# samuelskirvin/EIGENSOLVER

Hardware: AMD Instinct MI355X
Metric: det(M) evals/sec + roots/sec, 4096x4096 (k,omega) grid (higher is better)
Workload: dtype f64

## Files before the change

eigensolver_amd/build.py:

```python
import os
import shutil
import subprocess
import sys

HERE = os.path.dirname(os.path.abspath(__file__))
CSRC = os.path.join(HERE, "csrc")
LIBDIR = os.path.join(HERE, "lib")
LIB = os.path.join(LIBDIR, "libeigensolver_amd.so")
LIB_IEEE = os.path.join(LIBDIR, "libeigensolver_amd_ieee.so")
PROBE_SRC = os.path.join(os.path.dirname(HERE), "tests", "devmath", "devmath_probe.hip")
LIB_PROBE = os.path.join(LIBDIR, "libes_devmath_probe.so")
ARCH = "gfx950"
FLAGS = ["-O3", "-fPIC", "-std=c++17", f"--offload-arch={ARCH}", "-ffp-contract=off", "-fno-fast-math",
         "-Wall", "-Wno-unused-function", "-Wno-unused-result"]


def _hipcc():
    for c in (os.environ.get("HIPCC"), shutil.which("hipcc"), "/opt/rocm/bin/hipcc"):
        if c and os.path.exists(c):
            return c
    raise RuntimeError("hipcc not found (ROCm toolchain required)")


def sources():
    return sorted(os.path.join(CSRC, f) for f in os.listdir(CSRC) if f.endswith(".hip"))


def _deps():
    out = sources() + [os.path.join(CSRC, f) for f in os.listdir(CSRC) if f.endswith((".hpp", ".h"))]
    out.append(os.path.join(os.path.dirname(HERE), "include", "eigensolver_amd.h"))
    return out


def needs_build(lib=LIB):
    if not os.path.exists(lib):
        return True
    t = os.path.getmtime(lib)
    return any(os.path.getmtime(s) > t for s in _deps())


def _compile_and_link(lib, extra_flags, tag, verbose):
    hipcc = _hipcc()
    objs = []
    procs = []
    for src in sources():
        obj = os.path.join(LIBDIR, os.path.basename(src)[:-4] + tag + ".o")
        cmd = [hipcc] + FLAGS + extra_flags + ["-c", src, "-o", obj]
        if verbose:
            print(" ".join(cmd))
        procs.append((src, subprocess.Popen(cmd, stdout=subprocess.PIPE, stderr=subprocess.STDOUT, text=True)))
        objs.append(obj)
    for src, p in procs:
        out, _ = p.communicate()
        if p.returncode != 0:
            raise RuntimeError(f"hipcc failed for {src}:\n{out}")
        if verbose and out.strip():
            print(out)
    cmd = [hipcc, "-shared", "-fPIC", f"--offload-arch={ARCH}", "-o", lib] + objs
    r = subprocess.run(cmd, stdout=subprocess.PIPE, stderr=subprocess.STDOUT, text=True)
    if r.returncode != 0:
        raise RuntimeError(f"link failed:\n{r.stdout}")
    return lib


def _probe_needs_build():
    if not os.path.exists(LIB_PROBE):
        return True
    t = os.path.getmtime(LIB_PROBE)
    return any(os.path.getmtime(s) > t for s in (PROBE_SRC, os.path.join(CSRC, "es_bessel.hpp")))


def _build_probe(verbose):
    cmd = [_hipcc()] + FLAGS + ["-shared", PROBE_SRC, "-o", LIB_PROBE]
    if verbose:
        print(" ".join(cmd))
    r = subprocess.run(cmd, stdout=subprocess.PIPE, stderr=subprocess.STDOUT, text=True)
    if r.returncode != 0:
        raise RuntimeError(f"hipcc failed for {PROBE_SRC}:\n{r.stdout}")
    if verbose and r.stdout.strip():
        print(r.stdout)


def build(force=False, verbose=False):
    os.makedirs(LIBDIR, exist_ok=True)
    extra = ["-DES_ALL_GRID_SHAPES"] if os.environ.get("ES_BUILD_ALL_SHAPES") == "1" else []
    extra += os.environ.get("ES_BUILD_EXTRA_FLAGS", "").split()
    if force or needs_build(LIB):
        _compile_and_link(LIB, extra, "", verbose)
    if force or needs_build(LIB_IEEE):
        _compile_and_link(LIB_IEEE, ["-DES_IEEE_DIVISION"], ".ieee", verbose)
    if os.path.exists(PROBE_SRC) and (force or _probe_needs_build()):
        _build_probe(verbose)
    return LIB


if __name__ == "__main__":
    print(build(force="--force" in sys.argv, verbose=True))
```

eigensolver_amd/csrc/es_bessel.hpp:

```cpp
#pragma once
#include <math.h>

#ifndef ES_HD
#if defined(__HIPCC__)
#define ES_HD __host__ __device__ __forceinline__
#else
#define ES_HD static inline
#endif
#endif

namespace esb {

ES_HD double qdiv(double a, double b) {
#if defined(__HIP_DEVICE_COMPILE__) && !defined(ES_IEEE_DIVISION)
  const double r0 = __builtin_amdgcn_rcp(b);
  const double e = __builtin_fma(-b, r0, 1.0);
  const double t = __builtin_fma(e, e, e);
  return a * __builtin_fma(r0, t, r0);
#else
  return a / b;
#endif
}

#if defined(__HIP_DEVICE_COMPILE__) && !defined(ES_IEEE_DIVISION)
#define ES_BESSEL_TABLES 1
#define ES_R(k) (1.0 / (double)(k))
#define ES_R8(k) ES_R(k), ES_R((k) + 1), ES_R((k) + 2), ES_R((k) + 3), ES_R((k) + 4), ES_R((k) + 5), ES_R((k) + 6), ES_R((k) + 7)
#define ES_A(i) (1.0 / (-(((double)(i)) - 0.5) * (((double)(i)) - 0.5)))
#define ES_A8(i) ES_A(i), ES_A((i) + 1), ES_A((i) + 2), ES_A((i) + 3), ES_A((i) + 4), ES_A((i) + 5), ES_A((i) + 6), ES_A((i) + 7)
constexpr int kRcpTable = 64;
static __constant__ double kRcpInt[kRcpTable] = {0.0, ES_R(1), ES_R(2), ES_R(3), ES_R(4), ES_R(5), ES_R(6), ES_R(7), ES_R8(8), ES_R8(16),
                                                 ES_R8(24), ES_R8(32), ES_R8(40), ES_R8(48), ES_R8(56)};
static __constant__ double kRcpCF2a[kRcpTable] = {0.0, ES_A(1), ES_A(2), ES_A(3), ES_A(4), ES_A(5), ES_A(6), ES_A(7), ES_A8(8), ES_A8(16),
                                                  ES_A8(24), ES_A8(32), ES_A8(40), ES_A8(48), ES_A8(56)};
#undef ES_R
#undef ES_R8
#undef ES_A
#undef ES_A8
#endif

ES_HD double qdiv_int(double a, int k) {
#if defined(ES_BESSEL_TABLES)
  if (k < kRcpTable) return a * kRcpInt[k];
#endif
  return qdiv(a, (double)k);
}
ES_HD double qdiv_cf2a(double a, int i, double ai) {
#if defined(ES_BESSEL_TABLES)
  if (i < kRcpTable) return a * kRcpCF2a[i];
#endif
  return qdiv(a, ai);
}

constexpr double kEulerGamma = 0.57721566490153286060651209008240243;
constexpr double kPi = 3.14159265358979323846264338327950288;

#define ES_CHEB_K0 { \
    1.2201515410329777, -0.0314481013119645, 0.0015698838857300533, -0.00012849549581627802, \
    1.39498137188765e-05, -1.8317555227191195e-06, 2.766813639445015e-07, -4.660489897687948e-08, \
    8.574034017414225e-09, -1.6975345093890614e-09, 3.5773972814003283e-10, -7.957489244477396e-11, \
    1.8559491149549264e-11, -4.514597883374519e-12, 1.1403405882073441e-12, -2.9800969231481784e-13, \
    8.032890775068375e-14, -2.2275133267462965e-14, 6.340076476276646e-15, -1.848593377920907e-15, \
    5.5120559994043335e-16, -1.6782311257549006e-16, 5.2103917776435543e-17, -1.6475805939842632e-17, \
    5.3004337711773354e-18 }
#define ES_CHEB_K1 { \
    1.3603130952422213, 0.10392373657681724, -0.002857816859622779, 0.00019521551847135162, \
    -1.936197974166083e-05, 2.406484947837217e-06, -3.5019606030878126e-07, 5.7410841254500495e-08, \
    -1.0345762465678097e-08, 2.0150497551970347e-09, -4.1903547593419254e-10, 9.218315187605315e-11, \
    -2.129967838427791e-11, 5.139639673482343e-12, -1.2891739609498229e-12, 3.348419666052243e-13, \
    -8.976705182010146e-14, 2.4771544242195988e-14, -7.0198370892147685e-15, 2.038703166239861e-15, \
    -6.057047270643018e-16, 1.8380935752430455e-16, -5.689462849193648e-17, 1.7940510478863572e-17, \
    -5.7567444820733025e-18 }
constexpr int kChebN = 25;
#if defined(__HIP_DEVICE_COMPILE__)
static __constant__ double kChebK0[kChebN] = ES_CHEB_K0;
static __constant__ double kChebK1[kChebN] = ES_CHEB_K1;
#else
static const double kChebK0[kChebN] = ES_CHEB_K0;
static const double kChebK1[kChebN] = ES_CHEB_K1;
#endif

ES_HD void ke01(double x, double& k0, double& k1) {
  if (x <= 2.0) {
    const double t = 0.25 * x * x;
    const double lg = log(0.5 * x) + kEulerGamma;
    double term0 = 1.0, i0 = 1.0, s0 = 0.0, hk = 0.0;
    double term1 = 1.0, i1 = 1.0, s1 = 1.0;
    for (int k = 1; k < 40; ++k) {
      const double rk = qdiv_int(1.0, k), rk1 = qdiv_int(1.0, k + 1);
      term0 = term0 * t * (rk * rk);
      hk += rk;
      i0 += term0;
      s0 += hk * term0;
      term1 = term1 * t * (rk * rk1);
      i1 += term1;
      s1 += (hk + hk + rk1) * term1;
      if (term0 < 1e-18 * i0) break;
    }
    const double ex = exp(x);
    k0 = ex * (-lg * i0 + s0);
    k1 = ex * (qdiv(1.0, x) + lg * (0.5 * x) * i1 - 0.25 * x * s1);
  } else {
    const double y = qdiv(4.0, x) - 1.0, y2 = y + y;
    double p1 = 0.0, p2 = 0.0, q1 = 0.0, q2 = 0.0;
#pragma unroll
    for (int j = kChebN - 1; j >= 1; --j) {
      const double pn = fma(y2, p1, kChebK0[j] - p2);
      const double qn = fma(y2, q1, kChebK1[j] - q2);
      p2 = p1; p1 = pn;
      q2 = q1; q1 = qn;
    }
    const double rs = qdiv(1.0, sqrt(x));
    k0 = fma(y, p1, kChebK0[0] - p2) * rs;
    k1 = fma(y, q1, kChebK1[0] - q2) * rs;
  }
}

ES_HD void ke_pair(int n, double x, double& kn, double& knp1) {
  double a, b;
  ke01(x, a, b);
  const double tox = qdiv(2.0, x);
  for (int j = 1; j <= n; ++j) {
    const double c = a + (double)j * tox * b;
    a = b;
    b = c;
  }
  kn = a;
  knp1 = b;
}

ES_HD void ie_pair(int n, double x, double& in_, double& inp1) {
  const double t = 0.25 * x * x;
  const double hx = 0.5 * x;
  double pre = 1.0;
  for (int j = 1; j <= n; ++j) pre *= hx / (double)j;
  double term_a = 1.0, sum_a = 1.0;
  double term_b = 1.0, sum_b = 1.0;
  for (int k = 1; k < 400; ++k) {
    const double kk = (double)k;
    term_a = term_a * t / (kk * (kk + (double)n));
    term_b = term_b * t / (kk * (kk + (double)n + 1.0));
    sum_a += term_a;
    sum_b += term_b;
    if (term_a < 1e-18 * sum_a) break;
  }
  const double ex = exp(-x);
  in_ = ex * pre * sum_a;
  inp1 = ex * pre * (hx / ((double)n + 1.0)) * sum_b;
}

ES_HD void ie_pair_from_k(int n, double x, double kn, double knp1, double& in_, double& inp1) {
  if (x < 0.5) { ie_pair(n, x, in_, inp1); return; }
  const int M = n + 10 + (int)sqrt(40.0 * x);
  const double tox = 2.0 / x;
  double ip = 0.0, ic = 1e-200;
  double ktox = (double)M * tox;
  for (int k = M; k > n; --k) {
    const double im = fma(ktox, ic, ip);
    ip = ic;
    ic = im;
    ktox -= tox;
  }
  const double f = ip / ic;
  in_ = 1.0 / (x * fma(f, kn, knp1));
  inp1 = f * in_;
}

ES_HD void jy_pair(int n, double x, double& jn, double& jn1, double& yn, double& yn1) {
  int M = (int)(1.15 * x) + 36 + n;
  M += (M & 1);
  const double tox = 2.0 / x;
  double jp = 0.0, jc = 1e-280;
  double norm = 0.0, sy0 = 0.0, sy1 = 0.0;
  double rn = 0.0, rn1 = 0.0;
  for (int k = M; k >= 1; --k) {
    if (k == n) rn = jc;
    if (k == n + 1) rn1 = jc;
    const int h = k >> 1;
    const double sgn = (h & 1) ? -1.0 : 1.0;
    if ((k & 1) == 0) {
      norm += jc;
      sy0 -= sgn * jc / (double)h;
    } else if (k >= 3) {
      sy1 += sgn * (double)k * jc / ((double)h * (double)(h + 1));
    }
    const double jm = (double)k * tox * jc - jp;
    jp = jc;
    jc = jm;
    if (fabs(jc) > 1e250) {
      const double sc = 1e-250;
      jc *= sc; jp *= sc; norm *= sc; sy0 *= sc; sy1 *= sc; rn *= sc; rn1 *= sc;
    }
  }
  if (n == 0) rn = jc;
  if (n + 1 == 1) rn1 = jp;
  const double inv = 1.0 / (jc + 2.0 * norm);
  const double j0 = jc * inv, j1 = jp * inv;
  const double lg = log(0.5 * x) + kEulerGamma;
  const double y0 = (2.0 / kPi) * (lg * j0 + 2.0 * sy0 * inv);
// ... 15 lines not shown
```

eigensolver_amd/csrc/es_shoot.hip:

```cpp
#include <vector>
#include <cstdio>
#include <cstdlib>
#include <cmath>
#include <type_traits>

#include "es_shoot_shared.hpp"

namespace {
using namespace es_shoot_shared;

struct GridOpts {
  int skip;
  const int* cols;
  int part;
  int main_span;
};

constexpr long ES_TILE_GRID_X = 1L << 22;
__device__ __forceinline__ long es_tile_index() { return (long)blockIdx.y * ES_TILE_GRID_X + blockIdx.x; }
inline dim3 es_tile_grid(long tiles) {
  return tiles <= ES_TILE_GRID_X ? dim3((unsigned)tiles) : dim3((unsigned)ES_TILE_GRID_X, (unsigned)((tiles + ES_TILE_GRID_X - 1) / ES_TILE_GRID_X));
}

template <int FAM, int PTS, int MAXT, bool TRACK, int WPE = 0>
// ... 66 lines not shown
    const int j = (int)(c - row * nw);
    if (!dead[j]) continue;
    const double k = kv[row];
    const double w = k * wv[j];
    const double k2 = k * k;
    const double Oe = (P.family == FAM_CYL0 || P.family == FAM_CYLT) ? w : (w - k * P.U_e);
    const double Oe2 = Oe * Oe;
    const double m_e = ((k2 * P.vAe2 - Oe2) * (k2 * P.ce2 - Oe2)) / (P.Se * (k2 * P.cTe2 - Oe2));
    const double cst = (P.family == FAM_CYL0 || P.family == FAM_CYLT)
                           ? -1.0 / (P.rho_e * (k2 * P.vAe2 - w * w))
                           : P.rho_e * P.Se * (k2 * P.cTe2 - Oe2) / (Oe * (k2 * P.ce2 - Oe2));
    uint8_t st = ES_PT_CONTINUUM;
    if (m_e < 0.0) st = ES_PT_LEAKY;
    else if (!(m_e > 0.0) || !isfinite(m_e) || !isfinite(cst)) st = ES_PT_NONFINITE;
    Dout[c] = NAN;
    if (relout) relout[c] = NAN;
    stout[c] = st;
  }
}

template <int FAM>
__global__ __launch_bounds__(256) void shoot_points_kernel(ShootDev P, const double* __restrict__ kv,
                                                           const double* __restrict__ wv, const int* __restrict__ d_n,
                                                           int n_max, double* __restrict__ Dout,
                                                           double* __restrict__ relout, uint8_t* __restrict__ stout) {
  ES_POINT_LDS(FAM);
  const int n = es_count(d_n, n_max);
  if ((long)blockIdx.x * 256 >= (long)n) return;
  const int i = blockIdx.x * blockDim.x + threadIdx.x;
  const bool in = i < n;
  const double k = in ? kv[i] : 1.0;
  const double w = in ? wv[i] : 1.0;
  double D, rel; uint8_t st;
  shoot_point<FAM>(P, k, w, w, D, rel, st, es_point_lds);
  if (in) {
    Dout[i] = D;
    stout[i] = st;
    if (relout) relout[i] = rel;
  }
}

__global__ __launch_bounds__(256) void bracket_flag_kernel(const double* __restrict__ D,
                                                           const uint8_t* __restrict__ st, int nw, long cells,
                                                           uint64_t* __restrict__ masks,
                                                           int* __restrict__ block_counts) {
  __shared__ int wave_cnt[4];
  const long c = (long)blockIdx.x * 256 + threadIdx.x;
  const int lane = threadIdx.x & 63;
  double d0 = 0.0; int ok0 = 0;
  if (c < cells) { d0 = D[c]; ok0 = (st[c] == ES_PT_OK); }
  double d1 = __shfl_down(d0, 1);
  int ok1 = __shfl_down(ok0, 1);
  if (lane == 63) {
    if (c + 1 < cells) { d1 = D[c + 1]; ok1 = (st[c + 1] == ES_PT_OK); } else { d1 = 0.0; ok1 = 0; }
  }
  bool flag = false;
  if (c < cells) {
    const long row = c / nw;
    const int j = (int)(c - row * nw);
    flag = (j < nw - 1) && ok0 && ok1 && (d0 * d1 < 0.0);
  }
  const uint64_t m = __ballot(flag);
  if (lane == 0) {
    masks[c >> 6] = m;
    wave_cnt[threadIdx.x >> 6] = __popcll(m);
  }
  __syncthreads();
// ... 1690 lines not shown
```

eigensolver_amd/csrc/es_shoot_device.hpp:

```cpp
#pragma once
#include <hip/hip_runtime.h>
#include <math.h>
#include "es_bessel.hpp"
#include "../../include/eigensolver_amd.h"

enum { FAM_CYL0 = 0, FAM_CYLT = 1, FAM_SLABD = 2, FAM_SLABF = 3 };

struct ShootDev {
  int family;
  int n_nodes;
  int npts;
  double xb;
  double h;
  const double* base;
  double rho_e, vAe2, ce2, cTe2, Se, U_e;
  double R_factor;
  double ic0, ic1;
  int m, m_ext, axis_bc, c1_power;
  double bc_const;
  double bc_const_raw;
  double slab_sign;
  double c2_i, vA2_i, S_i, cT2_i, rho_i;
  int accept_norm;
  int use_bands, n_bands;
// ... 302 lines not shown
}

template <int FAM>
__device__ __forceinline__ void adjoint_step(double& p, double& q, const Coef& B0, const Coef& Bm, const Coef& B1,
                                             double h, double h2, double h6, double h3) {
  if (fam_unnormalised<FAM>()) rk4_step_adjoint_scaled0_x3(p, q, B0, Bm, B1);
  else if (fam_scaled<FAM>()) rk4_step_adjoint_scaled0(p, q, B0, Bm, B1);
  else rk4_step_adjoint<FamTraits<FAM>::SHAPE>(p, q, B0, Bm, B1, h, h2, h6, h3);
}

template <int FAM>
__device__ __forceinline__ void adjoint_step_normalised(double& p, double& q, const Coef& B0, const Coef& Bm, const Coef& B1,
                                                        double h, double h2, double h6, double h3) {
  if (fam_scaled<FAM>()) rk4_step_adjoint_scaled0(p, q, B0, Bm, B1);
  else rk4_step_adjoint<FamTraits<FAM>::SHAPE>(p, q, B0, Bm, B1, h, h2, h6, h3);
}

__device__ __forceinline__ void adjoint_start(const ShootDev& P, const Coef& A_last, double& p, double& q) {
  if ((P.family == FAM_CYL0 || P.family == FAM_CYLT) && P.axis_bc == ES_AXIS_SAUSAGE) {
    p = A_last.a11; q = A_last.a12;
  } else {
    p = 1.0; q = 0.0;
  }
}

struct Exterior {
  double m_e;
  double cst;
  double yb, dyb;
  double Oe;
  int status;
};

__device__ __forceinline__ Exterior exterior_cylinder(const ShootDev& P, double k, double w, double w_cst) {
  Exterior X;
  const double k2 = k * k, w2 = w * w;
  X.Oe = w;
  X.m_e = ((k2 * P.vAe2 - w2) * (k2 * P.ce2 - w2)) / (P.Se * (k2 * P.cTe2 - w2));
  X.cst = -1.0 / (P.rho_e * (k2 * P.vAe2 - w_cst * w_cst));
  X.yb = X.dyb = NAN;
  if (X.m_e < 0.0) { X.status = ES_PT_LEAKY; return X; }
  if (!(X.m_e > 0.0) || !isfinite(X.m_e) || !isfinite(X.cst)) { X.status = ES_PT_NONFINITE; return X; }
  X.status = ES_PT_OK;
  const double mu = sqrt(X.m_e);
  const double sgn = (P.xb < 0.0) ? -1.0 : 1.0;
  const double xR = mu * (P.R_factor / k), xb = mu;
  const int n = P.m_ext;
  double Kb, Kb1, KR, KR1;
  esb::ke_pair(n, xb, Kb, Kb1);
  esb::ke_pair(n, xR, KR, KR1);
  const double dn = (double)n;
  const double dKb = -Kb1 + (dn / xb) * Kb;
  const double dKR = -KR1 + (dn / xR) * KR;
  const double g = P.ic1 / (sgn * mu);
  double Pv, dPv;
  const double gap = xR - xb;
  if (gap < 40.0) {
    double Ib, Ib1, IR, IR1;
    esb::ie_pair_from_k(n, xb, Kb, Kb1, Ib, Ib1);
    esb::ie_pair_from_k(n, xR, KR, KR1, IR, IR1);
    const double dIb = Ib1 + (dn / xb) * Ib;
    const double dIR = IR1 + (dn / xR) * IR;
    const double a_s = -(P.ic0 * dKR - g * KR);
    const double b_s = -(g * IR - P.ic0 * dIR);
    const double E2 = exp(-2.0 * gap);
    Pv = b_s * Kb + E2 * a_s * Ib;
    dPv = sgn * mu * (b_s * dKb + E2 * a_s * dIb);
  } else {
    double IR, IR1;
    const double rI = 1.0 - 0.5 / xR - (4.0 * dn * dn - 1.0) / (8.0 * xR * xR);
    (void)IR; (void)IR1;
    const double b_s = -(g - P.ic0 * rI);
    Pv = b_s * Kb;
    dPv = sgn * mu * (b_s * dKb);
  }
  const double nrm = fabs(Pv);
  X.yb = Pv / nrm;
  X.dyb = dPv / nrm;
  if (!isfinite(X.yb) || !isfinite(X.dyb)) X.status = ES_PT_NONFINITE;
  return X;
}

__device__ __forceinline__ Exterior exterior_slab(const ShootDev& P, double k, double w) {
  Exterior X;
  const double k2 = k * k;
  const double Oe = w - k * P.U_e;
  const double Oe2 = Oe * Oe;
  X.Oe = Oe;
  X.m_e = ((k2 * P.vAe2 - Oe2) * (k2 * P.ce2 - Oe2)) / (P.Se * (k2 * P.cTe2 - Oe2));
  X.cst = P.rho_e * P.Se * (k2 * P.cTe2 - Oe2) / (Oe * (k2 * P.ce2 - Oe2));
  X.yb = X.dyb = NAN;
  if (X.m_e < 0.0) { X.status = ES_PT_LEAKY; return X; }
  if (!(X.m_e > 0.0) || !isfinite(X.m_e) || !isfinite(X.cst)) { X.status = ES_PT_NONFINITE; return X; }
  X.status = ES_PT_OK;
  const double mu = sqrt(X.m_e);
  const double R = P.R_factor / k;
  const double E2 = exp(-2.0 * mu * (R - 1.0));
  const double gp = P.ic0 + P.ic1 / mu, gm = P.ic0 - P.ic1 / mu;
  const double V = gp + E2 * gm;
  const double dV = mu * (gp - E2 * gm);
  const double nrm = fabs(V);
  X.yb = V / nrm;
  X.dyb = dV / nrm;
  if (!isfinite(X.yb) || !isfinite(X.dyb)) X.status = ES_PT_NONFINITE;
  return X;
}

struct Mismatch { double d, outer, inner; };

template <int FAM, class Ext>
__device__ __forceinline__ Mismatch boundary_algebra(const ShootDev& P, const KScal& s, double w, const Ext& X,
                                                     double r1, double r2, const double* e_first) {
  Mismatch M;
  if (FAM == FAM_CYL0 || FAM == FAM_CYLT) {
    const double Pb = X.yb;
    const double xi_e = X.outer;
    double Xb;
    if (P.axis_bc == ES_AXIS_KINK) {
      Xb = (P.bc_const * xi_e - r1 * Pb) / r2;
    } else if (P.axis_bc == ES_AXIS_ROTATION_KINK) {
      Xb = (-(P.bc_const * xi_e) - r1 * Pb) / r2;
    } else {
      Xb = -(r1 * Pb) / r2;
    }
    const double xi_i = Xb / P.xb;
    M.outer = xi_e; M.inner = xi_i; M.d = xi_e - xi_i;
  } else {
    const double P_left = X.outer;
    if (FAM == FAM_SLABD) {
      const double Vb = X.yb;
      const double sv = (P.slab_sign - r1) * Vb / r2;
      M.inner = sv / w;
    } else {
      const double Omb = w - e_first[0];
      const double Vb = X.yb * Omb / X.Oe;
      const double sv = (P.slab_sign - r1) * Vb / r2;
      const double Omb2 = Omb * Omb;
      const double PTi = P.rho_i * P.S_i * (s.kcT2 - Omb2) / (Omb * (s.kc2 - Omb2));
      M.inner = PTi * sv;
    }
    M.outer = P_left;
    M.d = P_left - M.inner;
  }
  return M;
}
```

eigensolver_amd/csrc/es_shoot_grid_body.hpp:

```cpp
  constexpr int NE = FamTraits<FAM>::NE;
  constexpr int LSTRIDE = 2 * CH + 2;
  constexpr bool PAIR = (FAM == FAM_CYL0) && !TRACK;
  constexpr bool STASH = (WPE != 0);
  __shared__ double xstash[STASH ? 4 * PTS * MAXT : 1];
  __shared__ __attribute__((aligned(16))) double lds_all[ROWS * NE * LSTRIDE];
  const int TW = blockDim.x;
  const int T = TW / ROWS;
  const int sub = (ROWS == 2 && (int)threadIdx.x >= T) ? 1 : 0;
  const int tl = (int)threadIdx.x - sub * T;
  const int tb = (ROWS == 2) ? sub * (NE * LSTRIDE) : 0;
  const int nsteps = P.n_nodes - 1;
  const double h = P.h, h2 = 0.5 * P.h, h6 = P.h / 6.0, h3 = P.h / 3.0;

  const int span = T * PTS;
  const int ncols = opts.cols ? opts.cols[0] : nw;
  const int col_base = (opts.part == 2) ? (ncols / opts.main_span) * opts.main_span : 0;
  const int nseg = (opts.part == 2) ? opts.main_span / span : (nw + span - 1) / span;
  const int ngroups = (nk + ROWS - 1) / ROWS;
  const long ntiles = (long)ngroups * nseg;
  for (long tile = es_tile_index(), once = 1; once && tile < ntiles; once = 0) {
    const int seg = (int)(tile / ngroups);
    const int grp = (int)(tile - (long)seg * ngroups);
    const bool row_ok = (ROWS == 1) || grp * ROWS + sub < nk;
    const int row = (ROWS == 1) ? grp : (row_ok ? grp * ROWS + sub : nk - 1);
    const int w0 = col_base + seg * span;
    if (w0 >= ncols) continue;
    if (opts.part == 1 && w0 + span > ncols) continue;
    const double k = kv[row];
    const KScal s = make_kscal(P, k);
    {
      double w[PTS], zp[PTS], zq[PTS];
      Coef B0[PTS], B1[PTS];
      SignTrack trk[PTS];
      bool inr[PTS];
      int iwp[PTS];
      ExteriorLite X[PTS];
      bool lane_live = false;
      if (STASH) {
#pragma unroll 1
        for (int p = 0; p < PTS; ++p) {
          const int ic = w0 + p * T + tl;
          const bool in = row_ok && ic < ncols;
          const int iw = in ? (opts.cols ? opts.cols[1 + ic] : ic) : 0;
          const double wp = in ? pick_w(wv, w_mode, k, row, nw, iw) : 1.0;
          const ExteriorLite Xp = exterior_lite(P, k, wp, wp);
          const bool dead = opts.skip && !TRACK && band_crossed(P, k, wp);
          lane_live = lane_live || (in && Xp.status == ES_PT_OK && !dead);
          double* xs = xstash + (size_t)(4 * p) * MAXT + threadIdx.x;
          xs[0] = Xp.outer; xs[MAXT] = Xp.yb; xs[2 * MAXT] = Xp.Oe; xs[3 * MAXT] = (double)Xp.status;
        }
      }
#pragma unroll
      for (int p = 0; p < PTS; ++p) {
        const int ic = w0 + p * T + tl;
        inr[p] = row_ok && ic < ncols;
        iwp[p] = inr[p] ? (opts.cols ? opts.cols[1 + ic] : ic) : 0;
        w[p] = inr[p] ? pick_w(wv, w_mode, k, row, nw, iwp[p]) : 1.0;
      }
      if (!STASH) {
#pragma unroll
        for (int p = 0; p < PTS; ++p) {
          X[p] = exterior_lite(P, k, w[p], w[p]);
          const bool dead = opts.skip && !TRACK && band_crossed(P, k, w[p]);
          lane_live = lane_live || (inr[p] && X[p].status == ES_PT_OK && !dead);
        }
      }
      const bool wave_live = __any(lane_live);
      const bool wg_live = __syncthreads_or(wave_live ? 1 : 0) != 0;
#pragma unroll
      for (int p = 0; p < PTS; ++p) { zp[p] = 0.0; zq[p] = 0.0; }
      const int nchunks = wg_live ? (nsteps + CH - 1) / CH : 0;
      for (int c = nchunks - 1; c >= 0; --c) {
        const int c0 = c * CH;
        const int nst = (nsteps - c0 < CH) ? (nsteps - c0) : CH;
        __syncthreads();
        const int nstage = 2 * nst + ES_FAR_NODE(c, nchunks);
        for (int i = threadIdx.x; i < ROWS * nstage; i += TW) {
          double b[FamTraits<FAM>::NB], e[NE];
          const int r = (ROWS == 2 && i >= nstage) ? 1 : 0;
          const int node = i - r * nstage;
          load_base<FAM>(P, 2 * c0 + node, b);
          if (ROWS == 1) {
            make_entry<FAM, fam_scaled<FAM>()>(b, s, e);
          } else {
            const int rr = grp * ROWS + r;
            const KScal sr = make_kscal(P, kv[rr < nk ? rr : nk - 1]);
            make_entry<FAM, fam_scaled<FAM>()>(b, sr, e);
          }
#pragma unroll
          for (int f = 0; f < NE; ++f) lds_all[r * (NE * LSTRIDE) + f * LSTRIDE + node] = e[f];
        }
        __syncthreads();
        if (!wave_live) continue;
        if (c == nchunks - 1) {
          double eL[NE];
// ... 67 lines not shown
            for (int p = 0; p < PTS; ++p) B0[p] = B1[p];
            --j;
          }
          for (; j >= 1; j -= 2) {
            ES_MARCH_STEP(j, B0, B1)
            ES_MARCH_STEP(j - 1, B1, B0)
          }
        } else {
          for (; j >= 0; --j) {
            ES_MARCH_STEP(j, B0, B1)
#pragma unroll
            for (int p = 0; p < PTS; ++p) B0[p] = B1[p];
          }
        }
#undef ES_MARCH_PAIR
#undef ES_MARCH_STEP
#pragma unroll
        for (int p = 0; p < PTS; ++p) adjoint_rescale<FAM>(zp[p], zq[p], nsteps - c0 - nst, nsteps - c0);
      }
      if (STASH) {
#pragma unroll
        for (int p = 0; p < PTS; ++p) {
          const double* xs = xstash + (size_t)(4 * p) * MAXT + threadIdx.x;
          X[p].outer = xs[0]; X[p].yb = xs[MAXT]; X[p].Oe = xs[2 * MAXT]; X[p].status = (int)xs[3 * MAXT];
        }
      }
      double bf[FamTraits<FAM>::NB], ef[NE];
      load_base<FAM>(P, 0, bf);
      make_entry<FAM>(bf, s, ef);
#pragma unroll
      for (int p = 0; p < PTS; ++p) {
        if (!inr[p]) continue;
        const int iw = iwp[p];
        const Mismatch M = boundary_algebra<FAM>(P, s, w[p], X[p], zp[p], zq[p], ef);
        double D, rel; uint8_t st;
        const bool crossed = TRACK ? trk[p].crossed() : band_crossed(P, k, w[p]);
        finish_point(P, M, X[p], crossed, D, rel, st);
        if (opts.skip && !TRACK && crossed && X[p].status == ES_PT_OK) st = ES_PT_CONTINUUM;
        if (opts.skip && st == ES_PT_CONTINUUM) { D = NAN; rel = NAN; }
        const size_t o = (size_t)row * nw + iw;
        Dout[o] = D;
        stout[o] = st;
        if (relout) relout[o] = rel;
      }
    }
  }
```

eigensolver_amd/csrc/es_shoot_shared.hpp:

```cpp
#pragma once
#include "es_common.hpp"
#include "es_shoot_device.hpp"

struct es_problem {
  ShootDev dev;
  double* d_base = nullptr;
  es_shoot_desc desc;
};

namespace es_shoot_shared {

constexpr int ES_REFINE_POLISH = 2;
#if defined(ES_STAGE_FAR_NODE_ALWAYS)
#define ES_FAR_NODE(c_, n_) 1
#else
#define ES_FAR_NODE(c_, n_) (((c_) == (n_) - 1) ? 1 : 0)
#endif
constexpr int CH = 128;

template <int FAM>
__device__ __forceinline__ void load_base(const ShootDev& P, int pt, double* b) {
#pragma unroll
  for (int f = 0; f < FamTraits<FAM>::NB; ++f) b[f] = P.base[(size_t)f * P.npts + pt];
}

__device__ __forceinline__ double pick_w(const double* __restrict__ wv, int w_mode, double k, int row, int nw, int iw) {
  if (w_mode == ES_W_PHASE_SPEED) return k * wv[iw];
  if (w_mode == ES_W_PER_ROW) return wv[(size_t)row * nw + iw];
  return wv[iw];
}

struct ExteriorLite {
  double outer, yb, Oe;
  int status;
};

__device__ __forceinline__ ExteriorLite exterior_lite(const ShootDev& P, double k, double w, double w_cst) {
  const Exterior X = (P.family == FAM_CYL0 || P.family == FAM_CYLT) ? exterior_cylinder(P, k, w, w_cst) : exterior_slab(P, k, w);
  ExteriorLite L;
  L.outer = X.cst * X.dyb;
  L.yb = X.yb;
  L.Oe = X.Oe;
  L.status = X.status;
  return L;
}

__device__ __forceinline__ void finish_point(const ShootDev& P, const Mismatch& M, const ExteriorLite& X, bool crossed,
                                             double& D, double& rel, uint8_t& st) {
  st = (uint8_t)X.status;
  D = M.d;
  const double sc = P.accept_norm ? fabs(M.outer) : fmax(fabs(M.outer), fabs(M.inner));
  rel = fabs(M.d) * 100.0 / sc;
  if (X.status != ES_PT_OK) { D = NAN; rel = NAN; return; }
  if (!isfinite(D)) { st = ES_PT_NONFINITE; return; }
  if (crossed) st = ES_PT_CONTINUUM;
}

template <int FAM, bool TRACK, bool BANDS = !TRACK, int C1P = 0>
__device__ __forceinline__ void shoot_point_impl(const ShootDev& P, double k, double w, double w_cst, double& D,
                                                 double& rel, uint8_t& st, double* __restrict__ sb) {
  constexpr int NE = FamTraits<FAM>::NE;
  constexpr int NB = FamTraits<FAM>::NB;
  const KScal s = make_kscal(P, k);
  const int nsteps = P.n_nodes - 1;
  const double h = P.h, h2 = 0.5 * P.h, h6 = P.h / 6.0, h3 = P.h / 3.0;
  SignTrack trk;
  double b[NB], e[NE], e2[NE];
  const ExteriorLite X = exterior_lite(P, k, w, w_cst);
  Coef B0;
  double zp = 0.0, zq = 0.0;
  const int nchunks = (nsteps + CH - 1) / CH;
  for (int c = nchunks - 1; c >= 0; --c) {
    const int c0 = c * CH;
    const int nst = (nsteps - c0 < CH) ? (nsteps - c0) : CH;
    __syncthreads();
#pragma unroll
    for (int f = 0; f < NB; ++f)
      for (int i = threadIdx.x; i < 2 * nst + ES_FAR_NODE(c, nchunks); i += blockDim.x)
        sb[i * NB + f] = P.base[(size_t)f * P.npts + 2 * c0 + i];
    __syncthreads();
    if (c == nchunks - 1) {
#pragma unroll
      for (int f = 0; f < NB; ++f) b[f] = sb[2 * nst * NB + f];
      make_entry<FAM, fam_scaled<FAM>()>(b, s, e);
      coefficients<FAM, TRACK, C1P>(e, P, s, w, B0, trk);
      adjoint_start(P, B0, zp, zq);
    }
#define ES_ENTRY(NODE, E)                                                                      \
    {                                                                                          \
      _Pragma("unroll") for (int f = 0; f < NB; ++f) b[f] = sb[(NODE) * NB + f];               \
      make_entry<FAM, fam_scaled<FAM>()>(b, s, E);                                             \
    }
    int j = nst - 1;
    if (fam_rcp4<FAM>()) {
      if (!(j & 1)) {
        Coef Bm, B1;
        ES_ENTRY(2 * j + 1, e)
        ES_ENTRY(2 * j, e2)
        coefficients2<FAM, TRACK, C1P>(e, e2, P, s, w, Bm, B1, trk);
        adjoint_step<FAM>(zp, zq, B0, Bm, B1, h, h2, h6, h3);
        B0 = B1;
// ... 13 lines not shown
          ES_ENTRY(2 * j - 4, e1)
          ES_ENTRY(2 * j - 5, em2)
          ES_ENTRY(2 * j - 6, e2)
          coefficients4<FAM, TRACK>(e, e1, em2, e2, P, s, w, Nm, N1, Nm2, N2, trk);
          adjoint_step<FAM>(zp, zq, B0, Cm, C1, h, h2, h6, h3);
          adjoint_step<FAM>(zp, zq, C1, Cm2, C2, h, h2, h6, h3);
          B0 = C2;
          Cm = Nm; C1 = N1; Cm2 = Nm2; C2 = N2;
        }
        adjoint_step<FAM>(zp, zq, B0, Cm, C1, h, h2, h6, h3);
        adjoint_step<FAM>(zp, zq, C1, Cm2, C2, h, h2, h6, h3);
        B0 = C2;
      }
    } else {
      Coef Cm, C1;
      ES_ENTRY(2 * j + 1, e)
      ES_ENTRY(2 * j, e2)
      coefficients2<FAM, TRACK, C1P>(e, e2, P, s, w, Cm, C1, trk);
      for (; j >= 1; --j) {
        Coef Nm, N1;
        ES_ENTRY(2 * j - 1, e)
        ES_ENTRY(2 * j - 2, e2)
        coefficients2<FAM, TRACK, C1P>(e, e2, P, s, w, Nm, N1, trk);
        adjoint_step<FAM>(zp, zq, B0, Cm, C1, h, h2, h6, h3);
        B0 = C1;
        Cm = Nm; C1 = N1;
      }
      adjoint_step<FAM>(zp, zq, B0, Cm, C1, h, h2, h6, h3);
      B0 = C1;
    }
#undef ES_ENTRY
    adjoint_rescale<FAM>(zp, zq, nsteps - c0 - nst, nsteps - c0);
  }
  const Mismatch M = boundary_algebra<FAM>(P, s, w, X, zp, zq, e2);
  finish_point(P, M, X, TRACK ? trk.crossed() : (BANDS ? band_crossed(P, k, w) : false), D, rel, st);
}

template <int FAM, bool TRACK, int CHR, int NG>
__device__ __forceinline__ void shoot_point_wavegroup_impl(const ShootDev& P, double k, double w, double& D, double& rel,
                                                           uint8_t& st, double* __restrict__ tbl) {
  constexpr int NE = FamTraits<FAM>::NE;
  constexpr int NB = FamTraits<FAM>::NB;
  constexpr int NODES = 2 * CHR + 1;
  constexpr int GL = 64 / NG;
  const int lane = threadIdx.x & 63;
  const int grp = lane / GL;
  const KScal s = make_kscal(P, k);
  const int nsteps = P.n_nodes - 1;
  const double h = P.h, h2 = 0.5 * P.h, h6 = P.h / 6.0, h3 = P.h / 3.0;
  SignTrack trk;
  double e[NE], e2[NE];
  const ExteriorLite X = exterior_lite(P, k, w, w);
  Coef B0;
  double zp = 0.0, zq = 0.0;
  const double* mine = tbl + (size_t)grp * NODES * NE;
  double kgs[NG];
#pragma unroll
  for (int g2 = 0; g2 < NG; ++g2) kgs[g2] = __shfl(k, g2 * GL);
  const int nchunks = (nsteps + CHR - 1) / CHR;
  for (int c = nchunks - 1; c >= 0; --c) {
    const int c0 = c * CHR;
    const int nst = (nsteps - c0 < CHR) ? (nsteps - c0) : CHR;
    const int nn = 2 * nst + ES_FAR_NODE(c, nchunks);
    __builtin_amdgcn_wave_barrier();
    for (int idx = lane; idx < NG * nn; idx += 64) {
      const int g2 = idx / nn, i = idx - g2 * nn;
      double kg = kgs[0];
// ... 34 lines not shown
        em2[f] = mine[(2 * j - 1) * NE + f]; e2[f] = mine[(2 * j - 2) * NE + f];
      }
      coefficients4<FAM, TRACK>(e, e1, em2, e2, P, s, w, Cm, C1, Cm2, C2, trk);
      for (; j >= 3; j -= 2) {
        Coef Nm, N1, Nm2, N2;
#pragma unroll
        for (int f = 0; f < NE; ++f) {
          e[f] = mine[(2 * j - 3) * NE + f]; e1[f] = mine[(2 * j - 4) * NE + f];
          em2[f] = mine[(2 * j - 5) * NE + f]; e2[f] = mine[(2 * j - 6) * NE + f];
        }
        coefficients4<FAM, TRACK>(e, e1, em2, e2, P, s, w, Nm, N1, Nm2, N2, trk);
        adjoint_step<FAM>(zp, zq, B0, Cm, C1, h, h2, h6, h3);
        adjoint_step<FAM>(zp, zq, C1, Cm2, C2, h, h2, h6, h3);
        B0 = C2;
        Cm = Nm; C1 = N1; Cm2 = Nm2; C2 = N2;
      }
      adjoint_step<FAM>(zp, zq, B0, Cm, C1, h, h2, h6, h3);
      adjoint_step<FAM>(zp, zq, C1, Cm2, C2, h, h2, h6, h3);
      B0 = C2;
    }
    adjoint_rescale<FAM>(zp, zq, nsteps - c0 - nst, nsteps - c0);
  }
  const Mismatch M = boundary_algebra<FAM>(P, s, w, X, zp, zq, e2);
  finish_point(P, M, X, TRACK ? trk.crossed() : band_crossed(P, k, w), D, rel, st);
}

template <int FAM, int CHR, int NG>
__device__ __forceinline__ void shoot_point_wavegroup(const ShootDev& P, double k, double w, double& D, double& rel,
                                                      uint8_t& st, double* __restrict__ tbl) {
  if (fam_has_bands<FAM>() && P.use_bands) shoot_point_wavegroup_impl<FAM, !fam_has_bands<FAM>(), CHR, NG>(P, k, w, D, rel, st, tbl);
  else shoot_point_wavegroup_impl<FAM, true, CHR, NG>(P, k, w, D, rel, st, tbl);
}

template <int FAM, bool STATUS = true>
__device__ __forceinline__ void shoot_point(const ShootDev& P, double k, double w, double w_cst, double& D,
                                            double& rel, uint8_t& st, double* __restrict__ sb) {
  if (FAM == FAM_CYLT) {
    if (!STATUS) {
      if (P.c1_power == 2) shoot_point_impl<FAM, false, false, 2>(P, k, w, w_cst, D, rel, st, sb);
      else shoot_point_impl<FAM, false, false, 1>(P, k, w, w_cst, D, rel, st, sb);
    } else {
      if (P.c1_power == 2) shoot_point_impl<FAM, true, false, 2>(P, k, w, w_cst, D, rel, st, sb);
      else shoot_point_impl<FAM, true, false, 1>(P, k, w, w_cst, D, rel, st, sb);
    }
  } else if (!STATUS) {
    shoot_point_impl<FAM, false, false>(P, k, w, w_cst, D, rel, st, sb);
  } else if (fam_has_bands<FAM>() && P.use_bands) shoot_point_impl<FAM, !fam_has_bands<FAM>()>(P, k, w, w_cst, D, rel, st, sb);
  else shoot_point_impl<FAM, true>(P, k, w, w_cst, D, rel, st, sb);
}

#define ES_POINT_LDS(FAM) __shared__ double es_point_lds[FamTraits<FAM>::NB * (2 * es_shoot_shared::CH + 1)]

}
```

Before: 869.7 million.

## Add fast cylinder exterior path with table-driven Bessel series and reciprocal division

Adds a fast exterior_cylinder variant that precomputes reciprocals of the Bessel arguments and shares them across K and I evaluation. The small-x K0/K1 series becomes Horner polynomials over a constexpr constant table. I_n is derived from K via a backward recurrence with a sqrt(x)-based start. Divisions in the exterior and boundary algebra go through an rcp+Newton qdiv with an IEEE fallback for extreme magnitudes. The aim is to cut per-point cost from transcendental and division work in the grid and point kernels, at the cost of last-bit accuracy differences and more code paths.

```diff
diff --git a/eigensolver_amd/build.py b/eigensolver_amd/build.py
--- a/eigensolver_amd/build.py
+++ b/eigensolver_amd/build.py
@@ -10,6 +10,8 @@
 LIB_IEEE = os.path.join(LIBDIR, "libeigensolver_amd_ieee.so")
 PROBE_SRC = os.path.join(os.path.dirname(HERE), "tests", "devmath", "devmath_probe.hip")
 LIB_PROBE = os.path.join(LIBDIR, "libes_devmath_probe.so")
+PROBE_FAST_SRC = os.path.join(os.path.dirname(HERE), "tests", "devmath", "exterior_fast_probe.hip")
+LIB_PROBE_FAST = os.path.join(LIBDIR, "libes_exterior_fast_probe.so")
 ARCH = "gfx950"
 FLAGS = ["-O3", "-fPIC", "-std=c++17", f"--offload-arch={ARCH}", "-ffp-contract=off", "-fno-fast-math",
          "-Wall", "-Wno-unused-function", "-Wno-unused-result"]
@@ -63,20 +65,20 @@
     return lib
 
 
-def _probe_needs_build():
-    if not os.path.exists(LIB_PROBE):
+def _probe_needs_build(src=PROBE_SRC, lib=LIB_PROBE):
+    if not os.path.exists(lib):
         return True
-    t = os.path.getmtime(LIB_PROBE)
-    return any(os.path.getmtime(s) > t for s in (PROBE_SRC, os.path.join(CSRC, "es_bessel.hpp")))
+    t = os.path.getmtime(lib)
+    return any(os.path.getmtime(s) > t for s in (src, os.path.join(CSRC, "es_bessel.hpp")))
 
 
-def _build_probe(verbose):
-    cmd = [_hipcc()] + FLAGS + ["-shared", PROBE_SRC, "-o", LIB_PROBE]
+def _build_probe(verbose, src=PROBE_SRC, lib=LIB_PROBE):
+    cmd = [_hipcc()] + FLAGS + ["-shared", src, "-o", lib]
     if verbose:
         print(" ".join(cmd))
     r = subprocess.run(cmd, stdout=subprocess.PIPE, stderr=subprocess.STDOUT, text=True)
     if r.returncode != 0:
-        raise RuntimeError(f"hipcc failed for {PROBE_SRC}:\n{r.stdout}")
+        raise RuntimeError(f"hipcc failed for {src}:\n{r.stdout}")
     if verbose and r.stdout.strip():
         print(r.stdout)
 
@@ -91,6 +93,8 @@
         _compile_and_link(LIB_IEEE, ["-DES_IEEE_DIVISION"], ".ieee", verbose)
     if os.path.exists(PROBE_SRC) and (force or _probe_needs_build()):
         _build_probe(verbose)
+    if os.path.exists(PROBE_FAST_SRC) and (force or _probe_needs_build(PROBE_FAST_SRC, LIB_PROBE_FAST)):
+        _build_probe(verbose, PROBE_FAST_SRC, LIB_PROBE_FAST)
     return LIB
 
 
diff --git a/eigensolver_amd/csrc/es_bessel.hpp b/eigensolver_amd/csrc/es_bessel.hpp
--- a/eigensolver_amd/csrc/es_bessel.hpp
+++ b/eigensolver_amd/csrc/es_bessel.hpp
@@ -51,6 +51,38 @@
 #endif
   return qdiv(a, ai);
 }
+
+ES_HD double rcp1(double x) { return qdiv(1.0, x); }
+
+#if defined(ES_BESSEL_TABLES)
+constexpr int kSerI0 = 12, kSerS0 = 12, kSerI1 = 11, kSerS1 = 12;
+struct KSeriesTable {
+  double i0[kSerI0 + 1], s0[kSerS0 + 1], i1[kSerI1 + 1], s1[kSerS1 + 1];
+};
+constexpr KSeriesTable make_kseries() {
+  KSeriesTable T{};
+  double fk = 1.0, hk = 0.0;
+  for (int k = 0; k <= 12; ++k) {
+    if (k > 0) { fk *= (double)k; hk += 1.0 / (double)k; }
+    const double fk1 = fk * (double)(k + 1), hk1 = hk + 1.0 / (double)(k + 1);
+    const double a = (1.0 / fk) / fk, b = (1.0 / fk) / fk1;
+    if (k <= kSerI0) T.i0[k] = a;
+    if (k <= kSerS0) T.s0[k] = hk * a;
+    if (k <= kSerI1) T.i1[k] = b;
+    if (k <= kSerS1) T.s1[k] = (hk + hk1) * b;
+  }
+  return T;
+}
+static __constant__ KSeriesTable kKSeries = make_kseries();
+
+#define ES_CONST_AS __attribute__((address_space(4)))
+template <class Tab>
+__device__ __forceinline__ const ES_CONST_AS Tab* local_table(const Tab* table) {
+  const ES_CONST_AS Tab* p = (const ES_CONST_AS Tab*)table;
+  asm volatile("" : "+s"(p));
+  return p;
+}
+#endif
 
 constexpr double kEulerGamma = 0.57721566490153286060651209008240243;
 constexpr double kPi = 3.14159265358979323846264338327950288;
@@ -80,6 +112,46 @@
 static const double kChebK1[kChebN] = ES_CHEB_K1;
 #endif
 
+#if defined(ES_BESSEL_TABLES)
+ES_HD void ke01(double x, double r, double& k0, double& k1, double& sx) {
+  if (x <= 2.0) {
+    const double t = 0.25 * x * x;
+    const double lg = log(0.5 * x) + kEulerGamma;
+    const ES_CONST_AS KSeriesTable* T = local_table(&kKSeries);
+    double i0 = T->i0[kSerI0], s0 = T->s0[kSerS0];
+#pragma unroll
+    for (int j = kSerI0 - 1; j >= 0; --j) i0 = fma(i0, t, T->i0[j]);
+#pragma unroll
+    for (int j = kSerS0 - 1; j >= 0; --j) s0 = fma(s0, t, T->s0[j]);
+    double i1 = T->i1[kSerI1], s1 = T->s1[kSerS1];
+#pragma unroll
+    for (int j = kSerI1 - 1; j >= 0; --j) i1 = fma(i1, t, T->i1[j]);
+#pragma unroll
+    for (int j = kSerS1 - 1; j >= 0; --j) s1 = fma(s1, t, T->s1[j]);
+    const double ex = exp(x);
+    k0 = ex * (-lg * i0 + s0);
+    k1 = ex * (r + lg * (0.5 * x) * i1 - 0.25 * x * s1);
+    sx = 1.4142135623730951;
+  } else {
+    const double y = 4.0 * r - 1.0, y2 = y + y;
+    double p1 = 0.0, p2 = 0.0, q1 = 0.0, q2 = 0.0;
+    const ES_CONST_AS double* c0 = local_table(&kChebK0[0]);
+    const ES_CONST_AS double* c1 = local_table(&kChebK1[0]);
+#pragma unroll
+    for (int j = kChebN - 1; j >= 1; --j) {
+      const double pn = fma(y2, p1, c0[j] - p2);
+      const double qn = fma(y2, q1, c1[j] - q2);
+      p2 = p1; p1 = pn;
+      q2 = q1; q1 = qn;
+    }
+    sx = sqrt(x);
+    const double rs = sx * r;
+    k0 = fma(y, p1, c0[0] - p2) * rs;
+    k1 = fma(y, q1, c1[0] - q2) * rs;
+  }
+}
+#endif
+
 ES_HD void ke01(double x, double& k0, double& k1) {
   if (x <= 2.0) {
     const double t = 0.25 * x * x;
@@ -129,6 +201,21 @@
   knp1 = b;
 }
 
+#if defined(ES_BESSEL_TABLES)
+ES_HD void ke_pair(int n, double x, double r, double& kn, double& knp1, double& sx) {
+  double a, b;
+  ke01(x, r, a, b, sx);
+  const double tox = 2.0 * r;
+  for (int j = 1; j <= n; ++j) {
+    const double c = a + (double)j * tox * b;
+    a = b;
+    b = c;
+  }
+  kn = a;
+  knp1 = b;
+}
+#endif
+
 ES_HD void ie_pair(int n, double x, double& in_, double& inp1) {
   const double t = 0.25 * x * x;
   const double hx = 0.5 * x;
@@ -165,6 +252,25 @@
   in_ = 1.0 / (x * fma(f, kn, knp1));
   inp1 = f * in_;
 }
+
+#if defined(ES_BESSEL_TABLES)
+ES_HD void ie_pair_from_k(int n, double x, double r, double sx, double kn, double knp1, double& in_, double& inp1) {
+  if (x < 0.5) { ie_pair(n, x, in_, inp1); return; }
+  const int M = n + 4 + (int)(6.324555320336759 * sx);
+  const double tox = 2.0 * r;
+  double ip = 0.0, ic = 1e-200;
+  double ktox = (double)M * tox;
+  for (int k = M; k > n; --k) {
+    const double im = fma(ktox, ic, ip);
+    ip = ic;
+    ic = im;
+    ktox -= tox;
+  }
+  const double f = qdiv(ip, ic);
+  in_ = rcp1(x * fma(f, kn, knp1));
+  inp1 = f * in_;
+}
+#endif
 
 ES_HD void jy_pair(int n, double x, double& jn, double& jn1, double& yn, double& yn1) {
   int M = (int)(1.15 * x) + 36 + n;
diff --git a/eigensolver_amd/csrc/es_shoot.hip b/eigensolver_amd/csrc/es_shoot.hip
--- a/eigensolver_amd/csrc/es_shoot.hip
+++ b/eigensolver_amd/csrc/es_shoot.hip
@@ -122,7 +122,7 @@
   const double k = in ? kv[i] : 1.0;
   const double w = in ? wv[i] : 1.0;
   double D, rel; uint8_t st;
-  shoot_point<FAM>(P, k, w, w, D, rel, st, es_point_lds);
+  shoot_point<FAM, true, true>(P, k, w, w, D, rel, st, es_point_lds);
   if (in) {
     Dout[i] = D;
     stout[i] = st;
diff --git a/eigensolver_amd/csrc/es_shoot_device.hpp b/eigensolver_amd/csrc/es_shoot_device.hpp
--- a/eigensolver_amd/csrc/es_shoot_device.hpp
+++ b/eigensolver_amd/csrc/es_shoot_device.hpp
@@ -358,6 +358,83 @@
   int status;
 };
 
+#if defined(__HIP_DEVICE_COMPILE__) && !defined(ES_IEEE_DIVISION)
+#define ES_FAST_EXTERIOR 1
+#endif
+
+template <bool FAST = true>
+__device__ __forceinline__ double status_div(double a, double b) {
+#if defined(ES_FAST_EXTERIOR)
+  if (FAST) {
+    const double q = esb::qdiv(a, b);
+    if (!(fabs(q) > 1e-290 && fabs(q) < 1e290)) return a / b;
+    return q;
+  }
+#endif
+  return a / b;
+}
+
+#if defined(ES_FAST_EXTERIOR)
+__device__ __forceinline__ Exterior exterior_cylinder_fast(const ShootDev& P, double k, double w, double w_cst) {
+  Exterior X;
+  const double k2 = k * k, w2 = w * w;
+  X.Oe = w;
+  X.m_e = status_div((k2 * P.vAe2 - w2) * (k2 * P.ce2 - w2), P.Se * (k2 * P.cTe2 - w2));
+  X.cst = status_div(-1.0, P.rho_e * (k2 * P.vAe2 - w_cst * w_cst));
+  X.yb = X.dyb = NAN;
+  if (X.m_e < 0.0) { X.status = ES_PT_LEAKY; return X; }
+  if (!(X.m_e > 0.0) || !isfinite(X.m_e) || !isfinite(X.cst)) { X.status = ES_PT_NONFINITE; return X; }
+  X.status = ES_PT_OK;
+  const double mu = sqrt(X.m_e);
+  const double sgn = (P.xb < 0.0) ? -1.0 : 1.0;
+  const double xR = mu * esb::qdiv(P.R_factor, k), xb = mu;
+  const double rb = esb::rcp1(xb), rR = esb::rcp1(xR);
+  const int n = P.m_ext;
+  double Kb, Kb1, KR, KR1, sxb, sxR;
+#if defined(ES_EXTERIOR_STUB)
+  if (ES_EXTERIOR_STUB & 1) { Kb = xb; Kb1 = rb; sxb = sqrt(xb); } else esb::ke_pair(n, xb, rb, Kb, Kb1, sxb);
+  if (ES_EXTERIOR_STUB & 2) { KR = xR; KR1 = rR; sxR = sqrt(xR); } else esb::ke_pair(n, xR, rR, KR, KR1, sxR);
+#else
+  esb::ke_pair(n, xb, rb, Kb, Kb1, sxb);
+  esb::ke_pair(n, xR, rR, KR, KR1, sxR);
+#endif
+  const double dn = (double)n;
+  const double nb = dn * rb, nR = dn * rR;
+  const double dKb = -Kb1 + nb * Kb;
+  const double dKR = -KR1 + nR * KR;
+  const double g = P.ic1 * (sgn * rb);
+  double Pv, dPv;
+  const double gap = xR - xb;
+  if (gap < 40.0) {
+    double Ib, Ib1, IR, IR1;
+#if defined(ES_EXTERIOR_STUB)
+    if (ES_EXTERIOR_STUB & 4) { Ib = rb; Ib1 = 0.5 * rb; IR = rR; IR1 = 0.5 * rR; } else
+#endif
+    {
+      esb::ie_pair_from_k(n, xb, rb, sxb, Kb, Kb1, Ib, Ib1);
+      esb::ie_pair_from_k(n, xR, rR, sxR, KR, KR1, IR, IR1);
+    }
+    const double dIb = Ib1 + nb * Ib;
+    const double dIR = IR1 + nR * IR;
+    const double a_s = -(P.ic0 * dKR - g * KR);
+    const double b_s = -(g * IR - P.ic0 * dIR);
+    const double E2 = exp(-2.0 * gap);
+    Pv = b_s * Kb + E2 * a_s * Ib;
+    dPv = sgn * mu * (b_s * dKb + E2 * a_s * dIb);
+  } else {
+    const double rI = 1.0 - 0.5 * rR - (4.0 * dn * dn - 1.0) * (0.125 * rR * rR);
+    const double b_s = -(g - P.ic0 * rI);
+    Pv = b_s * Kb;
+    dPv = sgn * mu * (b_s * dKb);
+  }
+  const double nrm = fabs(Pv);
+  X.yb = copysign(1.0, Pv);
+  X.dyb = status_div(dPv, nrm);
+  if (!(nrm > 0.0) || !isfinite(nrm) || !isfinite(X.dyb)) X.status = ES_PT_NONFINITE;
+  return X;
+}
+#endif
+
 __device__ __forceinline__ Exterior exterior_cylinder(const ShootDev& P, double k, double w, double w_cst) {
   Exterior X;
   const double k2 = k * k, w2 = w * w;
@@ -406,6 +483,11 @@
   if (!isfinite(X.yb) || !isfinite(X.dyb)) X.status = ES_PT_NONFINITE;
   return X;
 }
+#if !defined(ES_FAST_EXTERIOR)
+__device__ __forceinline__ Exterior exterior_cylinder_fast(const ShootDev& P, double k, double w, double w_cst) {
+  return exterior_cylinder(P, k, w, w_cst);
+}
+#endif
 
 __device__ __forceinline__ Exterior exterior_slab(const ShootDev& P, double k, double w) {
   Exterior X;
@@ -434,7 +516,7 @@
 
 struct Mismatch { double d, outer, inner; };
 
-template <int FAM, class Ext>
+template <int FAM, bool FAST = false, class Ext>
 __device__ __forceinline__ Mismatch boundary_algebra(const ShootDev& P, const KScal& s, double w, const Ext& X,
                                                      double r1, double r2, const double* e_first) {
   Mismatch M;
@@ -443,13 +525,13 @@
     const double xi_e = X.outer;
     double Xb;
     if (P.axis_bc == ES_AXIS_KINK) {
-      Xb = (P.bc_const * xi_e - r1 * Pb) / r2;
+      Xb = status_div<FAST>(P.bc_const * xi_e - r1 * Pb, r2);
     } else if (P.axis_bc == ES_AXIS_ROTATION_KINK) {
-      Xb = (-(P.bc_const * xi_e) - r1 * Pb) / r2;
+      Xb = status_div<FAST>(-(P.bc_const * xi_e) - r1 * Pb, r2);
     } else {
-      Xb = -(r1 * Pb) / r2;
+      Xb = status_div<FAST>(-(r1 * Pb), r2);
     }
-    const double xi_i = Xb / P.xb;
+    const double xi_i = status_div<FAST>(Xb, P.xb);
     M.outer = xi_e; M.inner = xi_i; M.d = xi_e - xi_i;
   } else {
     const double P_left = X.outer;
diff --git a/eigensolver_amd/csrc/es_shoot_grid_body.hpp b/eigensolver_amd/csrc/es_shoot_grid_body.hpp
--- a/eigensolver_amd/csrc/es_shoot_grid_body.hpp
+++ b/eigensolver_amd/csrc/es_shoot_grid_body.hpp
@@ -43,7 +43,7 @@
           const bool in = row_ok && ic < ncols;
           const int iw = in ? (opts.cols ? opts.cols[1 + ic] : ic) : 0;
           const double wp = in ? pick_w(wv, w_mode, k, row, nw, iw) : 1.0;
-          const ExteriorLite Xp = exterior_lite(P, k, wp, wp);
+          const ExteriorLite Xp = exterior_lite<FAM, true>(P, k, wp, wp);
           const bool dead = opts.skip && !TRACK && band_crossed(P, k, wp);
           lane_live = lane_live || (in && Xp.status == ES_PT_OK && !dead);
           double* xs = xstash + (size_t)(4 * p) * MAXT + threadIdx.x;
@@ -60,7 +60,7 @@
       if (!STASH) {
 #pragma unroll
         for (int p = 0; p < PTS; ++p) {
-          X[p] = exterior_lite(P, k, w[p], w[p]);
+          X[p] = exterior_lite<FAM, true>(P, k, w[p], w[p]);
           const bool dead = opts.skip && !TRACK && band_crossed(P, k, w[p]);
           lane_live = lane_live || (inr[p] && X[p].status == ES_PT_OK && !dead);
         }
@@ -194,7 +194,7 @@
       for (int p = 0; p < PTS; ++p) {
         if (!inr[p]) continue;
         const int iw = iwp[p];
-        const Mismatch M = boundary_algebra<FAM>(P, s, w[p], X[p], zp[p], zq[p], ef);
+        const Mismatch M = boundary_algebra<FAM, true>(P, s, w[p], X[p], zp[p], zq[p], ef);
         double D, rel; uint8_t st;
         const bool crossed = TRACK ? trk[p].crossed() : band_crossed(P, k, w[p]);
         finish_point(P, M, X[p], crossed, D, rel, st);
diff --git a/eigensolver_amd/csrc/es_shoot_shared.hpp b/eigensolver_amd/csrc/es_shoot_shared.hpp
--- a/eigensolver_amd/csrc/es_shoot_shared.hpp
+++ b/eigensolver_amd/csrc/es_shoot_shared.hpp
@@ -35,8 +35,11 @@
   int status;
 };
 
+template <int FAM = -1, bool FAST = false>
 __device__ __forceinline__ ExteriorLite exterior_lite(const ShootDev& P, double k, double w, double w_cst) {
-  const Exterior X = (P.family == FAM_CYL0 || P.family == FAM_CYLT) ? exterior_cylinder(P, k, w, w_cst) : exterior_slab(P, k, w);
+  const bool cyl = FAST ? (FAM == FAM_CYL0 || FAM == FAM_CYLT) : (P.family == FAM_CYL0 || P.family == FAM_CYLT);
+  const Exterior X = cyl ? (FAST ? exterior_cylinder_fast(P, k, w, w_cst) : exterior_cylinder(P, k, w, w_cst))
+                         : exterior_slab(P, k, w);
   ExteriorLite L;
   L.outer = X.cst * X.dyb;
   L.yb = X.yb;
@@ -56,7 +59,7 @@
   if (crossed) st = ES_PT_CONTINUUM;
 }
 
-template <int FAM, bool TRACK, bool BANDS = !TRACK, int C1P = 0>
+template <int FAM, bool TRACK, bool BANDS = !TRACK, int C1P = 0, bool FAST = false>
 __device__ __forceinline__ void shoot_point_impl(const ShootDev& P, double k, double w, double w_cst, double& D,
                                                  double& rel, uint8_t& st, double* __restrict__ sb) {
   constexpr int NE = FamTraits<FAM>::NE;
@@ -66,7 +69,7 @@
   const double h = P.h, h2 = 0.5 * P.h, h6 = P.h / 6.0, h3 = P.h / 3.0;
   SignTrack trk;
   double b[NB], e[NE], e2[NE];
-  const ExteriorLite X = exterior_lite(P, k, w, w_cst);
+  const ExteriorLite X = exterior_lite<FAM, FAST>(P, k, w, w_cst);
   Coef B0;
   double zp = 0.0, zq = 0.0;
   const int nchunks = (nsteps + CH - 1) / CH;
@@ -146,7 +149,7 @@
 #undef ES_ENTRY
     adjoint_rescale<FAM>(zp, zq, nsteps - c0 - nst, nsteps - c0);
   }
-  const Mismatch M = boundary_algebra<FAM>(P, s, w, X, zp, zq, e2);
+  const Mismatch M = boundary_algebra<FAM, FAST>(P, s, w, X, zp, zq, e2);
   finish_point(P, M, X, TRACK ? trk.crossed() : (BANDS ? band_crossed(P, k, w) : false), D, rel, st);
 }
 
@@ -247,21 +250,21 @@
   else shoot_point_wavegroup_impl<FAM, true, CHR, NG>(P, k, w, D, rel, st, tbl);
 }
 
-template <int FAM, bool STATUS = true>
+template <int FAM, bool STATUS = true, bool FAST = false>
 __device__ __forceinline__ void shoot_point(const ShootDev& P, double k, double w, double w_cst, double& D,
                                             double& rel, uint8_t& st, double* __restrict__ sb) {
   if (FAM == FAM_CYLT) {
     if (!STATUS) {
-      if (P.c1_power == 2) shoot_point_impl<FAM, false, false, 2>(P, k, w, w_cst, D, rel, st, sb);
-      else shoot_point_impl<FAM, false, false, 1>(P, k, w, w_cst, D, rel, st, sb);
+      if (P.c1_power == 2) shoot_point_impl<FAM, false, false, 2, FAST>(P, k, w, w_cst, D, rel, st, sb);
+      else shoot_point_impl<FAM, false, false, 1, FAST>(P, k, w, w_cst, D, rel, st, sb);
     } else {
-      if (P.c1_power == 2) shoot_point_impl<FAM, true, false, 2>(P, k, w, w_cst, D, rel, st, sb);
-      else shoot_point_impl<FAM, true, false, 1>(P, k, w, w_cst, D, rel, st, sb);
+      if (P.c1_power == 2) shoot_point_impl<FAM, true, false, 2, FAST>(P, k, w, w_cst, D, rel, st, sb);
+      else shoot_point_impl<FAM, true, false, 1, FAST>(P, k, w, w_cst, D, rel, st, sb);
     }
   } else if (!STATUS) {
-    shoot_point_impl<FAM, false, false>(P, k, w, w_cst, D, rel, st, sb);
-  } else if (fam_has_bands<FAM>() && P.use_bands) shoot_point_impl<FAM, !fam_has_bands<FAM>()>(P, k, w, w_cst, D, rel, st, sb);
-  else shoot_point_impl<FAM, true>(P, k, w, w_cst, D, rel, st, sb);
+    shoot_point_impl<FAM, false, false, 0, FAST>(P, k, w, w_cst, D, rel, st, sb);
+  } else if (fam_has_bands<FAM>() && P.use_bands) shoot_point_impl<FAM, !fam_has_bands<FAM>(), fam_has_bands<FAM>(), 0, FAST>(P, k, w, w_cst, D, rel, st, sb);
+  else shoot_point_impl<FAM, true, false, 0, FAST>(P, k, w, w_cst, D, rel, st, sb);
 }
 
 #define ES_POINT_LDS(FAM) __shared__ double es_point_lds[FamTraits<FAM>::NB * (2 * es_shoot_shared::CH + 1)]
```

Result: no change. 877.0 million (median of 6 runs) (+0.8%).
